# baumgach/PHiSeg-code

Hardware: AMD Instinct MI355X
Metric: training images/sec (ELBO step) phiseg_7_5 128x128 LIDC (higher is better)
Workload: dtype bf16; 1 GPU; phiseg_7_5 LIDC 128x128x1, 2 classes, bf16, batch norm, batch 64 per GPU, full ELBO training step (fwd + CE + KL + bwd + Adam); global_batch=64, parallelism=dp1

## Files before the change

### phiseg_code_amd/csrc/conv_c32.hip

```cpp
#include <stdlib.h>

#include <type_traits>

#include "phx_common.h"

namespace {

constexpr int C32_AI = 39;
constexpr int C32_NPL = 10;
constexpr int C32_STAGE = 40 * 1024;
constexpr int C32_PROW = 34 * 64;
constexpr int C32_LDS = 2 * C32_STAGE;

typedef __attribute__((address_space(3))) void* lds_ptr_t;

__device__ __forceinline__ unsigned lds_offset(const void* p) {
    return (unsigned)(uintptr_t)(const __attribute__((address_space(3))) unsigned char*)p;
}

__device__ unsigned long long* g_c32_trace = nullptr;
#define C32_TRACE(slot)                                                                          \
    do {                                                                                         \
        if (g_c32_trace && blockIdx.x == 0 && threadIdx.x == 0 && (slot) < 512)                   \
            g_c32_trace[slot] = __builtin_readcyclecounter();                                     \
    } while (0)

template <bool BIASACT, bool XF = false>
__global__ __launch_bounds__(256, 2) void k_conv3x3_c32(const unsigned short* __restrict__ x, const unsigned short* __restrict__ wpk,
                                                        unsigned short* __restrict__ y, const float* __restrict__ bias, int act,
                                                        float* __restrict__ stats_partial, int B, int H, int W, int tiles_x,
                                                        int tiles_y, int ntiles, const float* __restrict__ oscale, int stats_nrep, unsigned mgx, unsigned mgy,
                                                        const float* __restrict__ xscale = nullptr, const float* __restrict__ xshift = nullptr) {
    extern __shared__ __attribute__((aligned(16))) unsigned char smem[];
    const int wave = threadIdx.x >> 6, lane = threadIdx.x & 63;
    const int l31 = lane & 31, khalf = lane >> 5;

    bf16x8 fb[9][2];
#pragma unroll
    for (int tap = 0; tap < 9; ++tap)
#pragma unroll
        for (int ks = 0; ks < 2; ++ks)
            fb[tap][ks] = *reinterpret_cast<const bf16x8*>(wpk + ((tap * 32 + l31) * 32 + (ks * 2 + khalf) * 8));

    unsigned rel[C32_NPL], edge[C32_NPL];
#pragma unroll
    for (int n = 0; n < C32_NPL; ++n) {
        const int j = wave + 4 * n;
        const int e = j * 64 + lane, pp = e >> 2, slot = e & 3;
        const int py = pp / 34, px = pp - py * 34;
        rel[n] = (unsigned)((py * W + px) * 64 + ((slot ^ ((px >> 2) & 3)) << 4));
        edge[n] = (j < C32_AI && pp < 612) ? (unsigned)((px == 0) | ((px == 33) << 1) | ((py == 0) << 2) | ((py == 17) << 3)) : 15u;
    }
    const __amdgpu_buffer_rsrc_t rsx = __builtin_amdgcn_make_buffer_rsrc((void*)x, 0, (int)((unsigned)B * H * W * 64u), 0x00020000);
    auto decode = [&](int t, int* tx0, int* ty0, int* b0) {
        const int q1 = tiles_x == 1 ? t : (int)__umulhi((unsigned)t, mgx);
        *tx0 = (t - q1 * tiles_x) << 5;
// ... 248 lines not shown
```

### phiseg_code_amd/csrc/conv_wgrad.hip

```cpp
#include "conv_common.h"

template <int RB>
__device__ __forceinline__ int wswz(int pix, int byte_in_row) {
    if (RB == 128) return pix * 128 + (byte_in_row ^ (((pix >> 1) & 1) << 6));
    return pix * RB + byte_in_row;
}

template <int TCI, int TCO, bool BIGP, bool FAST16>
__device__ __forceinline__ void conv3x3_wgrad_body(const unsigned short* __restrict__ x0, const unsigned short* __restrict__ dy,
                                                   float* __restrict__ dw, float* __restrict__ ws, int B, int H, int W, int Cin,
                                                   int Cout, MTile g, int ntiles, int tiles_per_block, const int bx,
                                                   const int by, const int bz, const int gdx, const int gdy,
                                                   const unsigned short* __restrict__ x2 = nullptr, const int K1 = 0) {
    const bool src2 = x2 != nullptr && by * TCI >= K1;
    const unsigned short* __restrict__ x = src2 ? x2 : x0;
    const int xC = x2 == nullptr ? Cin : (src2 ? Cin - K1 : K1);
    const int xc0 = by * TCI - (src2 ? K1 : 0);
    constexpr int WI = TCI / 32, WJ = TCO / 32, WK = 4 / (WI * WJ);
    constexpr int RBX = TCI * 2, RBD = TCO * 2;
    constexpr int QX = TCI / 8, QD = TCO / 8;
    constexpr int NXI = ((BIGP ? 1024 : 400) * QX + 255) / 256;
    const int tw = 1 << g.tws, th = 1 << g.ths;
    const int pw = tw + 2, ph = th + 2;
    const int npatch = g.tb * ph * pw;
    extern __shared__ __attribute__((aligned(16))) unsigned char smem[];
    unsigned char* sX = smem;
    unsigned char* sD = smem + npatch * RBX;
    const int ci0 = by * TCI, co0 = bz * TCO;
    const int wave = threadIdx.x >> 6, lane = threadIdx.x & 63;
    const int wi = wave % WI, wj = (wave / WI) % WJ, wk = wave / (WI * WJ);
    const int c16 = lane & 15, cb16 = (lane >> 4) & 1, khalf = lane >> 5;
    const int chan_byte_x = (wi * 32 + cb16 * 16 + (c16 & 3) * 4) * 2;
    const int chan_byte_d = (wj * 32 + cb16 * 16 + (c16 & 3) * 4) * 2;
    typedef __attribute__((ext_vector_type(8))) short s16x8;
    unsigned dcon[2], xcon[2][3][2];
#pragma unroll
    for (int r = 0; r < 2; ++r) {
        const int lxr = khalf * 8 + r * 4 + (c16 >> 2);
        dcon[r] = (unsigned)wswz<RBD>(lxr, chan_byte_d);
#pragma unroll
// ... 65 lines not shown
        if constexpr (PHX_ABLATE & 16) return;
        if constexpr (idx < NXI) {
            const int gx = ptx0 + (planx[idx] & 255) - 1, gy = pty0 + ((planx[idx] >> 8) & 255) - 1, gb = pb0 + (planx[idx] >> 16);
            const bool ok = planx[idx] >= 0 && gx >= 0 && gx < W && gy >= 0 && gy < H && gb < B;
            const unsigned vo = ok ? (unsigned)(((gb * H + gy) * W + gx) * xC * 2 + qxb) : 0xffffffffu;
            rx[idx] = __builtin_amdgcn_raw_buffer_load_b128(rsx, vo, xc0 * 2, 0);
        } else if constexpr (idx < NXI + QD) {
            constexpr int it = idx - NXI;
            const int ox = ptx0 + (pland[it] & 255), oy = pty0 + ((pland[it] >> 8) & 255), ob = pb0 + (pland[it] >> 16);
            const bool ok = ox < W && oy < H && ob < B;
            const unsigned vo = ok ? (unsigned)(((ob * H + oy) * W + ox) * Cout * 2 + qdb) : 0xffffffffu;
            rd[it] = __builtin_amdgcn_raw_buffer_load_b128(rsd, vo, co0 * 2, 0);
        }
    };
    auto prefetch_range = [&](auto self, auto lo, auto hi) {
        constexpr int l = decltype(lo)::value, h = decltype(hi)::value;
        if constexpr (l < h && l < NXI + QD) {
            prefetch_piece(lo);
            self(self, std::integral_constant<int, l + 1>(), hi);
        }
    };
    const int t_begin = bx * tiles_per_block;
    const int t_end = min(ntiles, t_begin + tiles_per_block);
    PHX_BLOCKLOG_BEGIN();
    PHX_TRACE(0);
    if (t_begin < t_end) {
        if constexpr (FAST16) {
            decode(t_begin);
            prefetch_range(prefetch_range, std::integral_constant<int, 0>(), std::integral_constant<int, NXI + QD>());
        } else {
            prefetch(t_begin);
        }
    }
    PHX_TRACE(1);

    for (int t = t_begin; t < t_end; ++t) {
        __syncthreads();
        if (t == t_begin) PHX_TRACE(2);
#pragma unroll
        for (int it = 0; it < NXI; ++it) {
            const int i = threadIdx.x + it * 256;
            if (planx[it] >= 0) *reinterpret_cast<u32x4*>(sX + wswz<RBX>(i / QX, (i % QX) * 16)) = rx[it];
        }
#pragma unroll
        for (int it = 0; it < QD; ++it) {
            const int i = threadIdx.x + it * 256;
            *reinterpret_cast<u32x4*>(sD + wswz<RBD>(i / QD, (i % QD) * 16)) = rd[it];
        }
        __syncthreads();
        if (t == t_begin) PHX_TRACE(3);
        const bool more = t + 1 < t_end;
        if constexpr (FAST16) { if (more) decode(t + 1); }
        else if (more) prefetch(t + 1);
        if (t == t_begin) PHX_TRACE(4);
        if (FAST16) {
            constexpr int NSTEP = 16 / WK;
            s16x4 fd[2][2], fx[2][9][2];
            auto read_step = [&](unsigned xb, unsigned db, auto parc, auto bufc) {
                constexpr int P = decltype(parc)::value;
                constexpr int Bf = decltype(bufc)::value;
                fd[Bf][0] = __builtin_amdgcn_ds_read_tr16_b64_v4i16((s16x4 __attribute__((address_space(3)))*)(smem + db + dcon[0]));
                fd[Bf][1] = __builtin_amdgcn_ds_read_tr16_b64_v4i16((s16x4 __attribute__((address_space(3)))*)(smem + db + dcon[1]));
#pragma unroll
                for (int kh = 0; kh < 3; ++kh)
#pragma unroll
                    for (int kw = 0; kw < 3; ++kw) {
                        const int par = (P + kh) & 1;
                        fx[Bf][kh * 3 + kw][0] = __builtin_amdgcn_ds_read_tr16_b64_v4i16(
                            (s16x4 __attribute__((address_space(3)))*)(smem + xb + kh * 18 * RBX + xcon[0][kw][par]));
                        fx[Bf][kh * 3 + kw][1] = __builtin_amdgcn_ds_read_tr16_b64_v4i16(
                            (s16x4 __attribute__((address_space(3)))*)(smem + xb + kh * 18 * RBX + xcon[1][kw][par]));
                    }
            };
            auto mfma_step = [&](auto bufc) {
                constexpr int Bf = decltype(bufc)::value;
                const s16x8 dtmp = {fd[Bf][0][0], fd[Bf][0][1], fd[Bf][0][2], fd[Bf][0][3], fd[Bf][1][0], fd[Bf][1][1], fd[Bf][1][2], fd[Bf][1][3]};
                const bf16x8 bfrag = __builtin_bit_cast(bf16x8, dtmp);
// ... 46 lines not shown
                }
                const s16x4 d0 = __builtin_amdgcn_ds_read_tr16_b64_v4i16(
                    (s16x4 __attribute__((address_space(3)))*)(sD + wswz<RBD>(mpix[0], chan_byte_d)));
                const s16x4 d1 = __builtin_amdgcn_ds_read_tr16_b64_v4i16(
                    (s16x4 __attribute__((address_space(3)))*)(sD + wswz<RBD>(mpix[1], chan_byte_d)));
                const s16x8 dtmp = {d0[0], d0[1], d0[2], d0[3], d1[0], d1[1], d1[2], d1[3]};
                const bf16x8 bfrag = __builtin_bit_cast(bf16x8, dtmp);
    #pragma unroll
                for (int kh = 0; kh < 3; ++kh)
    #pragma unroll
                    for (int kw = 0; kw < 3; ++kw) {
                        const int sh = kh * pw + kw;
                        const s16x4 a0 = __builtin_amdgcn_ds_read_tr16_b64_v4i16(
                            (s16x4 __attribute__((address_space(3)))*)(sX + wswz<RBX>(ppix[0] + sh, chan_byte_x)));
                        const s16x4 a1 = __builtin_amdgcn_ds_read_tr16_b64_v4i16(
                            (s16x4 __attribute__((address_space(3)))*)(sX + wswz<RBX>(ppix[1] + sh, chan_byte_x)));
                        const s16x8 atmp = {a0[0], a0[1], a0[2], a0[3], a1[0], a1[1], a1[2], a1[3]};
                        const bf16x8 afrag = __builtin_bit_cast(bf16x8, atmp);
                        acc[kh * 3 + kw] = __builtin_amdgcn_mfma_f32_32x32x16_bf16(afrag, bfrag, acc[kh * 3 + kw], 0, 0, 0);
                    }
            }
        }
    }
    PHX_TRACE(5);
    if (ws) {
        const size_t cb = (size_t)bz * gdy + by;
        float* wp = ws + ((cb * gdx + bx) * WK + wk) * (size_t)(9 * TCI * TCO);
#pragma unroll
        for (int k = 0; k < 9; ++k)
#pragma unroll
            for (int r = 0; r < 16; ++r) {
                const int cil = wi * 32 + (r & 3) + 8 * (r >> 2) + 4 * (lane >> 5);
                wp[(k * TCI + cil) * TCO + wj * 32 + (lane & 31)] = acc[k][r];
            }
    } else {
        const int co = co0 + wj * 32 + (lane & 31);
#pragma unroll
        for (int k = 0; k < 9; ++k)
#pragma unroll
            for (int r = 0; r < 16; ++r) {
                const int ci = ci0 + wi * 32 + (r & 3) + 8 * (r >> 2) + 4 * (lane >> 5);
                atomicAdd(&dw[((size_t)k * Cin + ci) * Cout + co], acc[k][r]);
            }
    }
    PHX_TRACE(6);
    PHX_BLOCKLOG_END();
}

template <int TCI, int TCO, bool BIGP, bool FAST16>
__global__ __launch_bounds__(256, 1) void k_conv3x3_wgrad(const unsigned short* __restrict__ x,
                                                          const unsigned short* __restrict__ dy,
                                                          float* __restrict__ dw, float* __restrict__ ws, int B, int H,
                                                          int W, int Cin, int Cout, MTile g, int ntiles,
                                                          int tiles_per_block, const unsigned short* __restrict__ x2, int K1) {
    conv3x3_wgrad_body<TCI, TCO, BIGP, FAST16>(x, dy, dw, ws, B, H, W, Cin, Cout, g, ntiles, tiles_per_block, blockIdx.x,
                                               blockIdx.y, blockIdx.z, gridDim.x, gridDim.y, x2, K1);
}
struct WgMJob {
    const unsigned short* x; const unsigned short* dy; float* dw; float* ws;
    int B, H, W, Cin, Cout;
    MTile g;
    int ntiles, tpb, gdx, gdy, gdz, blk0;
    const unsigned short* x2; int K1, pad_;
};
template <int TCI, int TCO, bool BIGP>
__global__ __launch_bounds__(256, 1) void k_conv3x3_wgrad_multi(const WgMJob* __restrict__ jobs, int njobs) {
    int lo = 0, hi = njobs - 1;
    while (lo < hi) {
        const int mid = (lo + hi + 1) >> 1;
        if (jobs[mid].blk0 <= (int)blockIdx.x) lo = mid; else hi = mid - 1;
    }
    const WgMJob j = jobs[lo];
    const int local = blockIdx.x - j.blk0;
    conv3x3_wgrad_body<TCI, TCO, BIGP, false>(j.x, j.dy, j.dw, j.ws, j.B, j.H, j.W, j.Cin, j.Cout, j.g, j.ntiles, j.tpb,
                                              local % j.gdx, (local / j.gdx) % j.gdy, local / (j.gdx * j.gdy), j.gdx, j.gdy, j.x2, j.K1);
}

template <int TCI, int TCO>
__device__ __forceinline__ void conv3x3_wgrad_dma_body(const unsigned short* __restrict__ x0, const unsigned short* __restrict__ dy,
                                                       float* __restrict__ ws, int B, int H, int W, int Cin, int Cout, MTile g,
                                                       int ntiles, int tiles_per_block, const int bx, const int by, const int bz,
                                                       const int gdx, const int gdy,
                                                       const unsigned short* __restrict__ x2 = nullptr, const int K1 = 0,
                                                       const float* __restrict__ xscale = nullptr, const float* __restrict__ xshift = nullptr) {
    const bool src2 = x2 != nullptr && by * TCI >= K1;
    const unsigned short* __restrict__ x = src2 ? x2 : x0;
    const int xC = x2 == nullptr ? Cin : (src2 ? Cin - K1 : K1);
    const int xc0 = by * TCI - (src2 ? K1 : 0);
    constexpr int WI = TCI / 32, WJ = TCO / 32, WK = 4 / (WI * WJ);
    constexpr int RBX = TCI * 2, RBD = TCO * 2;
    constexpr int QX = TCI / 8, QD = TCO / 8;
    constexpr int NPATCH = 324;
    constexpr int XI = (NPATCH * QX + 63) / 64, DI = 256 * QD / 64;
    constexpr int XN = (XI + 3) / 4, DN = DI / 4;
    constexpr int SD_OFF = XI * 1024;
    extern __shared__ __attribute__((aligned(16))) unsigned char smem[];
    const int ci0 = by * TCI, co0 = bz * TCO;
    const int wave = threadIdx.x >> 6, lane = threadIdx.x & 63;
    const int wi = wave % WI, wj = (wave / WI) % WJ, wk = wave / (WI * WJ);
    const int c16 = lane & 15, cb16 = (lane >> 4) & 1, khalf = lane >> 5;
    const int chan_byte_x = (wi * 32 + cb16 * 16 + (c16 & 3) * 4) * 2;
    const int chan_byte_d = (wj * 32 + cb16 * 16 + (c16 & 3) * 4) * 2;
    typedef __attribute__((ext_vector_type(8))) short s16x8;
    unsigned dcon[2], xcon[2][3][2];
#pragma unroll
    for (int r = 0; r < 2; ++r) {
        const int lxr = khalf * 8 + r * 4 + (c16 >> 2);
        dcon[r] = (unsigned)(SD_OFF + wswz<RBD>(lxr, chan_byte_d));
#pragma unroll
        for (int kw = 0; kw < 3; ++kw)
#pragma unroll
            for (int par = 0; par < 2; ++par)
                xcon[r][kw][par] = (unsigned)((lxr + kw) * RBX +
                                              (RBX == 128 ? (chan_byte_x ^ (((((lxr + kw) >> 1) & 1) ^ par) << 6)) : chan_byte_x));
    }
    f32x16 acc[9];
#pragma unroll
    for (int k = 0; k < 9; ++k)
#pragma unroll
        for (int r = 0; r < 16; ++r) acc[k][r] = 0.f;

    constexpr bool RPLAN = WK == 1;
    auto plan_x = [&](int n) -> int {
        const int e = (wave + 4 * n) * 64 + lane;
        const int pp = e / QX, ps = e % QX;
        const int p = RBX == 128 ? (ps ^ (((pp >> 1) & 1) << 2)) : ps;
        return pp < NPATCH ? ((pp % 18) | ((pp / 18) << 8) | (p << 16)) : -1;
    };
    auto plan_d = [&](int n) -> int {
        const int e = (wave + 4 * n) * 64 + lane;
        const int m = e / QD, ps = e % QD;
        const int p = RBD == 128 ? (ps ^ (((m >> 1) & 1) << 2)) : ps;
        return (m & 15) | ((m >> 4) << 8) | (p << 16);
    };
    int planx[RPLAN ? XN : 1], pland[RPLAN ? DN : 1];
    if constexpr (RPLAN) {
#pragma unroll
        for (int n = 0; n < XN; ++n) planx[n] = plan_x(n);
#pragma unroll
        for (int n = 0; n < DN; ++n) pland[n] = plan_d(n);
    }
    const __amdgpu_buffer_rsrc_t rsx = __builtin_amdgcn_make_buffer_rsrc((void*)x, 0, (int)((unsigned)B * H * W * xC * 2u), 0x00020000);
    const __amdgpu_buffer_rsrc_t rsd = __builtin_amdgcn_make_buffer_rsrc((void*)dy, 0, (int)((unsigned)B * H * W * Cout * 2u), 0x00020000);
    typedef __attribute__((address_space(3))) void* lds_ptr_t;

    const int t_begin = bx * tiles_per_block;
    const int t_end = min(ntiles, t_begin + tiles_per_block);
    PHX_BLOCKLOG_BEGIN();
    for (int t = t_begin; t < t_end; ++t) {
        int tt = t;
        const int tx0 = (tt % g.tiles_x) << 4; tt /= g.tiles_x;
        const int ty0 = (tt % g.tiles_y) << 4; tt /= g.tiles_y;
        const int b0 = tt;
        __syncthreads();
#pragma unroll
        for (int n = 0; n < XN; ++n) {
            if (wave + 4 * n < XI) {
                int pk;
                if constexpr (RPLAN) pk = planx[n]; else pk = plan_x(n);
                const int gx = tx0 + (pk & 255) - 1, gy = ty0 + ((pk >> 8) & 255) - 1;
                const bool ok = pk >= 0 && gx >= 0 && gx < W && gy >= 0 && gy < H;
                const unsigned vo = ok ? (unsigned)((((b0 * H + gy) * W + gx) * xC) * 2 + (pk >> 16) * 16) : 0xffffffffu;
                __builtin_amdgcn_raw_ptr_buffer_load_lds(rsx, (lds_ptr_t)(smem + (wave + 4 * n) * 1024), 16, vo, xc0 * 2, 0, 0);
            }
        }
#pragma unroll
        for (int n = 0; n < DN; ++n) {
            int pk;
            if constexpr (RPLAN) pk = pland[n]; else pk = plan_d(n);
            const int ox = tx0 + (pk & 255), oy = ty0 + ((pk >> 8) & 255);
            const bool ok = ox < W && oy < H;
            const unsigned vo = ok ? (unsigned)((((b0 * H + oy) * W + ox) * Cout) * 2 + (pk >> 16) * 16) : 0xffffffffu;
            __builtin_amdgcn_raw_ptr_buffer_load_lds(rsd, (lds_ptr_t)(smem + SD_OFF + (wave + 4 * n) * 1024), 16, vo, co0 * 2, 0, 0);
        }
        asm volatile("s_waitcnt vmcnt(0)" ::: "memory");
        __syncthreads();
        if constexpr (TCI == 32) {
            if (xscale != nullptr) {
                typedef __attribute__((ext_vector_type(4))) unsigned u32x4_t;
                typedef __attribute__((ext_vector_type(4))) float f32x4_t;
                const int sp = threadIdx.x & 3;
                const f32x4_t c0 = *reinterpret_cast<const f32x4_t*>(xscale + ci0 + sp * 8), c1 = *reinterpret_cast<const f32x4_t*>(xscale + ci0 + sp * 8 + 4);
                const f32x4_t d0 = *reinterpret_cast<const f32x4_t*>(xshift + ci0 + sp * 8), d1 = *reinterpret_cast<const f32x4_t*>(xshift + ci0 + sp * 8 + 4);
                const float xsc[8] = {c0[0], c0[1], c0[2], c0[3], c1[0], c1[1], c1[2], c1[3]};
                const float xsh[8] = {d0[0], d0[1], d0[2], d0[3], d1[0], d1[1], d1[2], d1[3]};
#pragma unroll
                for (int n = 0; n < 6; ++n) {
                    const int pp = (int)(threadIdx.x >> 2) + 64 * n;
                    if (pp < NPATCH) {
                        const int py = (int)(((unsigned)pp * 3641u) >> 16), px = pp - py * 18;
                        const int gx = tx0 + px - 1, gy = ty0 + py - 1;
                        const bool inside = gx >= 0 && gx < W && gy >= 0 && gy < H;
                        u32x4_t* const q = reinterpret_cast<u32x4_t*>(smem + pp * RBX + sp * 16);
                        const u32x4_t r = *q;
                        u32x4_t o;
#pragma unroll
                        for (int k = 0; k < 4; ++k) {
                            const float a0 = fmaxf(fmaf(__uint_as_float(r[k] << 16), xsc[2 * k], xsh[2 * k]), 0.f);
                            const float a1 = fmaxf(fmaf(__uint_as_float(r[k] & 0xffff0000u), xsc[2 * k + 1], xsh[2 * k + 1]), 0.f);
                            o[k] = inside ? f2bf_pk(a0, a1) : 0u;
                        }
                        *q = o;
                    }
                }
                __syncthreads();
            }
        }

        constexpr int NSTEP = 16 / WK;
        s16x4 fd[2][2], fx[2][9][2];
        auto read_step = [&](unsigned xb, unsigned db, auto parc, auto bufc) {
            constexpr int P = decltype(parc)::value;
            constexpr int Bf = decltype(bufc)::value;
            fd[Bf][0] = __builtin_amdgcn_ds_read_tr16_b64_v4i16((s16x4 __attribute__((address_space(3)))*)(smem + db + dcon[0]));
            fd[Bf][1] = __builtin_amdgcn_ds_read_tr16_b64_v4i16((s16x4 __attribute__((address_space(3)))*)(smem + db + dcon[1]));
#pragma unroll
            for (int kh = 0; kh < 3; ++kh)
#pragma unroll
                for (int kw = 0; kw < 3; ++kw) {
                    const int par = (P + kh) & 1;
                    fx[Bf][kh * 3 + kw][0] = __builtin_amdgcn_ds_read_tr16_b64_v4i16(
                        (s16x4 __attribute__((address_space(3)))*)(smem + xb + kh * 18 * RBX + xcon[0][kw][par]));
                    fx[Bf][kh * 3 + kw][1] = __builtin_amdgcn_ds_read_tr16_b64_v4i16(
                        (s16x4 __attribute__((address_space(3)))*)(smem + xb + kh * 18 * RBX + xcon[1][kw][par]));
                }
        };
        auto mfma_step = [&](auto bufc) {
            constexpr int Bf = decltype(bufc)::value;
            const s16x8 dtmp = {fd[Bf][0][0], fd[Bf][0][1], fd[Bf][0][2], fd[Bf][0][3], fd[Bf][1][0], fd[Bf][1][1], fd[Bf][1][2], fd[Bf][1][3]};
            const bf16x8 bfrag = __builtin_bit_cast(bf16x8, dtmp);
#pragma unroll
            for (int k = 0; k < 9; ++k) {
                const s16x8 atmp = {fx[Bf][k][0][0], fx[Bf][k][0][1], fx[Bf][k][0][2], fx[Bf][k][0][3],
                                    fx[Bf][k][1][0], fx[Bf][k][1][1], fx[Bf][k][1][2], fx[Bf][k][1][3]};
                acc[k] = __builtin_amdgcn_mfma_f32_32x32x16_bf16(__builtin_bit_cast(bf16x8, atmp), bfrag, acc[k], 0, 0, 0);
            }
        };
        const unsigned xw = (unsigned)(wk * NSTEP * 18 * RBX), dw_ = (unsigned)(wk * NSTEP * 16 * RBD);
        read_step(xw, dw_, std::integral_constant<int, 0>(), std::integral_constant<int, 0>());
        auto steps = [&](auto self, auto stepc) {
            constexpr int SI = decltype(stepc)::value;
            if constexpr (SI < NSTEP) {
                if constexpr (SI + 1 < NSTEP)
                    read_step(xw + (SI + 1) * 18 * RBX, dw_ + (SI + 1) * 16 * RBD, std::integral_constant<int, (SI + 1) & 1>(),
                              std::integral_constant<int, (SI + 1) & 1>());
                mfma_step(std::integral_constant<int, SI & 1>());
                __builtin_amdgcn_sched_barrier(0);
                self(self, std::integral_constant<int, SI + 1>());
            }
        };
        steps(steps, std::integral_constant<int, 0>());
    }
    if constexpr (WK > 1) {
        typedef __attribute__((ext_vector_type(4))) float f32x4_t;
        f32x4_t* red = reinterpret_cast<f32x4_t*>(smem);
#pragma unroll
        for (int half = 1; half < WK; half <<= 1) {
            const int sel = wk & (2 * half - 1);
            f32x4_t* p = red + (size_t)(wi + WI * (wj + WJ * (wk / (2 * half)))) * (9 * 4 * 64) + lane;
            __syncthreads();
            if (sel == half)
#pragma unroll
                for (int k = 0; k < 9; ++k)
#pragma unroll
                    for (int q = 0; q < 4; ++q)
                        p[(k * 4 + q) * 64] = f32x4_t{acc[k][4 * q], acc[k][4 * q + 1], acc[k][4 * q + 2], acc[k][4 * q + 3]};
            __syncthreads();
            if (sel == 0)
#pragma unroll
                for (int k = 0; k < 9; ++k)
#pragma unroll
                    for (int q = 0; q < 4; ++q) {
                        const f32x4_t v = p[(k * 4 + q) * 64];
                        acc[k][4 * q] += v[0]; acc[k][4 * q + 1] += v[1]; acc[k][4 * q + 2] += v[2]; acc[k][4 * q + 3] += v[3];
                    }
        }
    }
    if (WK == 1 || wk == 0) {
        const size_t cb = (size_t)bz * gdy + by;
        float* wp = ws + (cb * gdx + bx) * (size_t)(9 * TCI * TCO);
#pragma unroll
        for (int k = 0; k < 9; ++k)
#pragma unroll
            for (int r = 0; r < 16; ++r) {
                const int cil = wi * 32 + (r & 3) + 8 * (r >> 2) + 4 * (lane >> 5);
                wp[(k * TCI + cil) * TCO + wj * 32 + (lane & 31)] = acc[k][r];
            }
    }
    PHX_BLOCKLOG_END();
}

template <int TCI, int TCO>
__global__ __launch_bounds__(256, 2) void k_conv3x3_wgrad_dma(const unsigned short* __restrict__ x,
                                                              const unsigned short* __restrict__ dy, float* __restrict__ ws,
                                                              int B, int H, int W, int Cin, int Cout, MTile g, int ntiles,
                                                              int tiles_per_block, const unsigned short* __restrict__ x2, int K1,
                                                              const float* __restrict__ xscale, const float* __restrict__ xshift) {
    conv3x3_wgrad_dma_body<TCI, TCO>(x, dy, ws, B, H, W, Cin, Cout, g, ntiles, tiles_per_block, blockIdx.x, blockIdx.y, blockIdx.z,
                                     gridDim.x, gridDim.y, x2, K1, xscale, xshift);
}
template <int TCI, int TCO>
__global__ __launch_bounds__(256, 2) void k_conv3x3_wgrad_dma_multi(const WgMJob* __restrict__ jobs, int njobs) {
    int lo = 0, hi = njobs - 1;
    while (lo < hi) {
        const int mid = (lo + hi + 1) >> 1;
        if (jobs[mid].blk0 <= (int)blockIdx.x) lo = mid; else hi = mid - 1;
    }
    const WgMJob j = jobs[lo];
    const int local = blockIdx.x - j.blk0;
    conv3x3_wgrad_dma_body<TCI, TCO>(j.x, j.dy, j.ws, j.B, j.H, j.W, j.Cin, j.Cout, j.g, j.ntiles, j.tpb, local % j.gdx,
                                     (local / j.gdx) % j.gdy, local / (j.gdx * j.gdy), j.gdx, j.gdy, j.x2, j.K1);
}

__device__ __forceinline__ void conv3x3_wgrad_pp_body(const unsigned short* __restrict__ x0, const unsigned short* __restrict__ dy,
                                                      float* __restrict__ ws, int B, int H, int W, int Cin, int Cout, MTile g,
                                                      int ntiles, int tiles_per_block, const int bx, const int by, const int bz,
                                                      const int gdx, const int gdy,
                                                      const unsigned short* __restrict__ x2 = nullptr, const int K1 = 0) {
    constexpr int TCI = 64, TCO = 64;
    const bool src2 = x2 != nullptr && by * TCI >= K1;
    const unsigned short* __restrict__ x = src2 ? x2 : x0;
    const int xC = x2 == nullptr ? Cin : (src2 ? Cin - K1 : K1);
    const int xc0 = by * TCI - (src2 ? K1 : 0);
    constexpr int RBX = 128, RBD = 128, QX = 8, QD = 8, NPATCH = 324;
    constexpr int XI = (NPATCH * QX + 63) / 64, DI = 256 * QD / 64;
    constexpr int XN = (XI + 3) / 4, DN = DI / 4;
    constexpr int SD_OFF = XI * 1024, STAGE = SD_OFF + 256 * RBD;
    extern __shared__ __attribute__((aligned(16))) unsigned char smem[];
    const int co0 = bz * TCO;
    const int wave = __builtin_amdgcn_readfirstlane((int)(threadIdx.x >> 6)), lane = threadIdx.x & 63;
    const int half = wave >> 2, lw = wave & 3;
    const int wi = lw & 1, wj = lw >> 1;
    const unsigned sbase = (unsigned)(half * STAGE);
    typedef __attribute__((ext_vector_type(8))) short s16x8;
    unsigned dcon[2], xcon[2][3][2];
    {
        const int c16 = lane & 15, cb16 = (lane >> 4) & 1, khalf = lane >> 5;
        const int chan_byte_x = (wi * 32 + cb16 * 16 + (c16 & 3) * 4) * 2;
        const int chan_byte_d = (wj * 32 + cb16 * 16 + (c16 & 3) * 4) * 2;
#pragma unroll
        for (int r = 0; r < 2; ++r) {
            const int lxr = khalf * 8 + r * 4 + (c16 >> 2);
// ... 79 lines not shown
                auto slot = [&](auto kc) {
                    constexpr int k = decltype(kc)::value, kh = k / 3, kw = k % 3, Rs = (SI + kh) & 3;
                    const s16x8 atmp = {fx[Rs][kw][0][0], fx[Rs][kw][0][1], fx[Rs][kw][0][2], fx[Rs][kw][0][3],
                                        fx[Rs][kw][1][0], fx[Rs][kw][1][1], fx[Rs][kw][1][2], fx[Rs][kw][1][3]};
                    acc[k] = __builtin_amdgcn_mfma_f32_32x32x16_bf16(__builtin_bit_cast(bf16x8, atmp), bfrag, acc[k], 0, 0, 0);
                    if constexpr (more) {
                        if constexpr (k < 2) rd_d(IC(SI + 1), kc);
                        else if constexpr (k < 8) rd_x(IC(SI + 3), IC((k - 2) >> 1), IC((k - 2) & 1));
                    }
                    __builtin_amdgcn_sched_barrier(0);
                };
                slot(IC(0)); slot(IC(1)); slot(IC(2)); slot(IC(3)); slot(IC(4)); slot(IC(5)); slot(IC(6)); slot(IC(7)); slot(IC(8));
                self(self, IC(SI + 1));
            }
        };
        steps(steps, IC(0));
#undef IC
    };
#define WPP_BARRIER() asm volatile("s_waitcnt vmcnt(0) lgkmcnt(0)\n\ts_barrier" ::: "memory")
    const int t_begin = bx * tiles_per_block;
    const int t_end = min(ntiles, t_begin + tiles_per_block);
    const int n = t_end - t_begin;
    const int nA = (n + 1) >> 1, nh = half ? (n >> 1) : nA;
    PHX_BLOCKLOG_BEGIN();
    if (half == 0 && nh > 0) load_tile(t_begin);
    WPP_BARRIER();
    if (half) {
        if (nh > 0) load_tile(t_begin + 1);
        WPP_BARRIER();
    }
    for (int k = 0; k < nA; ++k) {
        if (k < nh) compute();
        WPP_BARRIER();
        if (k + 1 < nh) load_tile(t_begin + half + 2 * (k + 1));
        WPP_BARRIER();
    }
    if (half == 0) WPP_BARRIER();
    typedef __attribute__((ext_vector_type(4))) float f32x4_t;
    f32x4_t* const pr = reinterpret_cast<f32x4_t*>(smem) + (size_t)lw * (9 * 4 * 64) + lane;
    if (half)
#pragma unroll
        for (int k = 0; k < 9; ++k)
#pragma unroll
            for (int q = 0; q < 4; ++q) pr[(k * 4 + q) * 64] = f32x4_t{acc[k][4 * q], acc[k][4 * q + 1], acc[k][4 * q + 2], acc[k][4 * q + 3]};
    WPP_BARRIER();
#undef WPP_BARRIER
    if (half == 0) {
        const size_t cb = (size_t)bz * gdy + by;
        float* wp = ws + (cb * gdx + bx) * (size_t)(9 * TCI * TCO);
#pragma unroll
        for (int k = 0; k < 9; ++k) {
#pragma unroll
            for (int q = 0; q < 4; ++q) {
                const f32x4_t v = pr[(k * 4 + q) * 64];
                acc[k][4 * q] += v[0]; acc[k][4 * q + 1] += v[1]; acc[k][4 * q + 2] += v[2]; acc[k][4 * q + 3] += v[3];
            }
#pragma unroll
            for (int r = 0; r < 16; ++r) {
                const int cil = wi * 32 + (r & 3) + 8 * (r >> 2) + 4 * (lane >> 5);
                wp[(k * TCI + cil) * TCO + wj * 32 + (lane & 31)] = acc[k][r];
            }
        }
    }
    PHX_BLOCKLOG_END();
}

__global__ __launch_bounds__(512, 1) void k_conv3x3_wgrad_pp(const unsigned short* __restrict__ x, const unsigned short* __restrict__ dy,
                                                             float* __restrict__ ws, int B, int H, int W, int Cin, int Cout, MTile g,
                                                             int ntiles, int tiles_per_block, const unsigned short* __restrict__ x2,
                                                             int K1) {
    conv3x3_wgrad_pp_body(x, dy, ws, B, H, W, Cin, Cout, g, ntiles, tiles_per_block, blockIdx.x, blockIdx.y, blockIdx.z, gridDim.x,
                          gridDim.y, x2, K1);
}
__global__ __launch_bounds__(512, 1) void k_conv3x3_wgrad_pp_multi(const WgMJob* __restrict__ jobs, int njobs) {
    int lo = 0, hi = njobs - 1;
    while (lo < hi) {
        const int mid = (lo + hi + 1) >> 1;
        if (jobs[mid].blk0 <= (int)blockIdx.x) lo = mid; else hi = mid - 1;
    }
    const WgMJob j = jobs[lo];
    const int local = blockIdx.x - j.blk0;
    const int cb = j.gdy * j.gdz, t = local >> 3;
    const int c = t % cb, bx = (t / cb) * 8 + (local & 7);
    if (bx >= j.gdx) return;
    conv3x3_wgrad_pp_body(j.x, j.dy, j.ws, j.B, j.H, j.W, j.Cin, j.Cout, j.g, j.ntiles, j.tpb, bx, c % j.gdy, c / j.gdy, j.gdx, j.gdy,
                          j.x2, j.K1);
}
// ... 42 lines not shown
    int lo = 0, hi = njobs - 1;
    while (lo < hi) {
        const int mid = (lo + hi + 1) >> 1;
        if (jobs[mid].blk0 <= (int)blockIdx.x) lo = mid; else hi = mid - 1;
    }
    const WgrJob j = jobs[lo];
    const int local = blockIdx.x - j.blk0;
    wgrad_reduce_body(j.ws, j.dw, j.nslice, j.Cin, j.Cout, j.tci, j.tco, local % j.gx, local / j.gx, j.gy);
}


int phx_wgrad_set_debug(void* trace_buf, void* blocklog_buf, int which) {
    unsigned long long* p = (unsigned long long*)(which == 0 ? trace_buf : blocklog_buf);
    if (which == 0) PHX_CHECK_HIP(hipMemcpyToSymbol(HIP_SYMBOL(g_phx_trace), &p, sizeof(p)));
    else PHX_CHECK_HIP(hipMemcpyToSymbol(HIP_SYMBOL(g_phx_blocklog), &p, sizeof(p)));
    return PHX_OK;
}

extern "C" {

static bool wgrad_dma_enabled() { return true; }
static size_t wgrad_dma_lds(int tci, int tco) {
    if (tci == 64 && tco == 64) return (size_t)2 * (41 * 1024 + 256 * 128);
    const size_t stage = (size_t)((324 * (tci / 8) + 63) / 64) * 1024 + (size_t)256 * tco * 2;
    const size_t red = (tci == 64 && tco == 64) ? 0 : (size_t)2 * 9 * 16 * 64 * sizeof(float);
    return stage > red ? stage : red;
}
static int wgrad_plan(int B, int H, int W, int Cin, int Cout, MTile* g, int* tci, int* tco, int* gx, int* tpb, int* wk,
                      int target_override = 0, int K1 = 0) {
    *g = make_mtile(B, H, W);
    const int ntiles = g->tiles_x * g->tiles_y * g->tiles_b;
    *tci = Cin % 64 == 0 ? 64 : 32;
    if (K1 > 0 && K1 % 64 != 0) *tci = 32;
    *tco = Cout % 64 == 0 ? 64 : 32;
    *wk = 4 / ((*tci / 32) * (*tco / 32));
    if (wgrad_dma_enabled() && g->tws == 4 && g->ths == 4 && g->tb == 1) *wk = 1;
    const int cblocks = (Cin / *tci) * (Cout / *tco);
    int target_blocks = cblocks <= 4 && *tci == 64 && *tco == 64 ? 512 : 384;
    if (ntiles <= 256 && target_blocks > 256) target_blocks = 256;
    const bool pp = wgrad_dma_enabled() && g->tws == 4 && g->ths == 4 && g->tb == 1 && *tci == 64 && *tco == 64;
    if (pp) target_blocks = 256;
    if (target_override > 0) target_blocks = pp ? (target_override + 1) / 2 : target_override;
    int split = (target_blocks + cblocks - 1) / cblocks;
    if (pp && target_override <= 0) split = target_blocks / cblocks;
    if (pp && target_override > 0) {
        const int alone = 256 / cblocks > 0 ? 256 / cblocks : 1;
        split = (split + 7) & ~7;
// ... 239 lines not shown
```

Baseline: 6756 images/s.

## Double-buffer DMA wgrad tiles and tighten LDS addressing with immediate offsets

New measurement: 6807 images/s, median of 6. Within noise of the previous version (+0.8%).

```diff
diff --git a/phiseg_code_amd/csrc/conv_c32.hip b/phiseg_code_amd/csrc/conv_c32.hip
--- a/phiseg_code_amd/csrc/conv_c32.hip
+++ b/phiseg_code_amd/csrc/conv_c32.hip
@@ -21,8 +21,7 @@
 __device__ unsigned long long* g_c32_trace = nullptr;
 #define C32_TRACE(slot)                                                                          \
     do {                                                                                         \
-        if (g_c32_trace && blockIdx.x == 0 && threadIdx.x == 0 && (slot) < 512)                   \
-            g_c32_trace[slot] = __builtin_readcyclecounter();                                     \
+        if (trc != nullptr && threadIdx.x == 0 && (slot) < 512) trc[slot] = __builtin_readcyclecounter(); \
     } while (0)
 
 template <bool BIASACT, bool XF = false>
@@ -32,6 +31,7 @@
                                                         int tiles_y, int ntiles, const float* __restrict__ oscale, int stats_nrep, unsigned mgx, unsigned mgy,
                                                         const float* __restrict__ xscale = nullptr, const float* __restrict__ xshift = nullptr) {
     extern __shared__ __attribute__((aligned(16))) unsigned char smem[];
+    unsigned long long* const trc = blockIdx.x == 0 ? g_c32_trace : nullptr;
     const int wave = threadIdx.x >> 6, lane = threadIdx.x & 63;
     const int l31 = lane & 31, khalf = lane >> 5;
 
diff --git a/phiseg_code_amd/csrc/conv_wgrad.hip b/phiseg_code_amd/csrc/conv_wgrad.hip
--- a/phiseg_code_amd/csrc/conv_wgrad.hip
+++ b/phiseg_code_amd/csrc/conv_wgrad.hip
@@ -16,6 +16,9 @@
     const unsigned short* __restrict__ x = src2 ? x2 : x0;
     const int xC = x2 == nullptr ? Cin : (src2 ? Cin - K1 : K1);
     const int xc0 = by * TCI - (src2 ? K1 : 0);
+    const unsigned long long trv = (unsigned long long)g_phx_trace, blv = (unsigned long long)g_phx_blocklog;
+    asm volatile("" ::: "memory");
+    unsigned long long *trc = nullptr, *blg = nullptr;
     constexpr int WI = TCI / 32, WJ = TCO / 32, WK = 4 / (WI * WJ);
     constexpr int RBX = TCI * 2, RBD = TCO * 2;
     constexpr int QX = TCI / 8, QD = TCO / 8;
@@ -127,8 +130,7 @@
     };
     const int t_begin = bx * tiles_per_block;
     const int t_end = min(ntiles, t_begin + tiles_per_block);
-    PHX_BLOCKLOG_BEGIN();
-    PHX_TRACE(0);
+    const unsigned long long bl_t0 = __builtin_readcyclecounter();
     if (t_begin < t_end) {
         if constexpr (FAST16) {
             decode(t_begin);
@@ -137,11 +139,14 @@
             prefetch(t_begin);
         }
     }
-    PHX_TRACE(1);
+    blg = phx_uniform_ptr(blv);
+    trc = (blockIdx.x | blockIdx.y | blockIdx.z) == 0 ? phx_uniform_ptr(trv) : nullptr;
+    PHX_TRACE_TO(trc, 0, bl_t0);
+    PHX_TRACE_TO(trc, 1, __builtin_readcyclecounter());
 
     for (int t = t_begin; t < t_end; ++t) {
         __syncthreads();
-        if (t == t_begin) PHX_TRACE(2);
+        if (t == t_begin) PHX_TRACE_TO(trc, 2, __builtin_readcyclecounter());
 #pragma unroll
         for (int it = 0; it < NXI; ++it) {
             const int i = threadIdx.x + it * 256;
@@ -153,11 +158,11 @@
             *reinterpret_cast<u32x4*>(sD + wswz<RBD>(i / QD, (i % QD) * 16)) = rd[it];
         }
         __syncthreads();
-        if (t == t_begin) PHX_TRACE(3);
+        if (t == t_begin) PHX_TRACE_TO(trc, 3, __builtin_readcyclecounter());
         const bool more = t + 1 < t_end;
         if constexpr (FAST16) { if (more) decode(t + 1); }
         else if (more) prefetch(t + 1);
-        if (t == t_begin) PHX_TRACE(4);
+        if (t == t_begin) PHX_TRACE_TO(trc, 4, __builtin_readcyclecounter());
         if (FAST16) {
             constexpr int NSTEP = 16 / WK;
             s16x4 fd[2][2], fx[2][9][2];
@@ -250,7 +255,7 @@
             }
         }
     }
-    PHX_TRACE(5);
+    PHX_TRACE_TO(trc, 5, __builtin_readcyclecounter());
     if (ws) {
         const size_t cb = (size_t)bz * gdy + by;
         float* wp = ws + ((cb * gdx + bx) * WK + wk) * (size_t)(9 * TCI * TCO);
@@ -271,8 +276,8 @@
                 atomicAdd(&dw[((size_t)k * Cin + ci) * Cout + co], acc[k][r]);
             }
     }
-    PHX_TRACE(6);
-    PHX_BLOCKLOG_END();
+    PHX_TRACE_TO(trc, 6, __builtin_readcyclecounter());
+    PHX_BLOCKLOG_END_TO(blg);
 }
 
 template <int TCI, int TCO, bool BIGP, bool FAST16>
@@ -304,6 +309,18 @@
                                               local % j.gdx, (local / j.gdx) % j.gdy, local / (j.gdx * j.gdy), j.gdx, j.gdy, j.x2, j.K1);
 }
 
+#ifndef PHX_WGRAD_DMA_STAGES
+#define PHX_WGRAD_DMA_STAGES 0
+#endif
+constexpr int wgrad_dma_xstages(int tci, int tco) {
+    return PHX_WGRAD_DMA_STAGES == 1 ? 1 : PHX_WGRAD_DMA_STAGES == 2 ? 2 : PHX_WGRAD_DMA_STAGES == 3 ? (tci == 32 ? 2 : 1) : (tci == 32 && tco == 32 ? 2 : 1);
+}
+constexpr int wgrad_dma_dstages(int tci, int tco) {
+    return PHX_WGRAD_DMA_STAGES == 1 ? 1 : PHX_WGRAD_DMA_STAGES == 2 ? 2 : PHX_WGRAD_DMA_STAGES == 3 ? (tco == 32 ? 2 : 1) : (tci == 32 && tco == 32 ? 2 : 1);
+}
+__device__ __forceinline__ unsigned wg_lds_offset(const void* p) {
+    return (unsigned)(uintptr_t)(const __attribute__((address_space(3))) unsigned char*)p;
+}
 template <int TCI, int TCO>
 __device__ __forceinline__ void conv3x3_wgrad_dma_body(const unsigned short* __restrict__ x0, const unsigned short* __restrict__ dy,
                                                        float* __restrict__ ws, int B, int H, int W, int Cin, int Cout, MTile g,
@@ -321,26 +338,33 @@
     constexpr int NPATCH = 324;
     constexpr int XI = (NPATCH * QX + 63) / 64, DI = 256 * QD / 64;
     constexpr int XN = (XI + 3) / 4, DN = DI / 4;
-    constexpr int SD_OFF = XI * 1024;
+    constexpr int XS = wgrad_dma_xstages(TCI, TCO), DS = wgrad_dma_dstages(TCI, TCO);
+    constexpr bool PIPE = XS == 2 || DS == 2;
+    constexpr int XSTAGE = XI * 1024, DSTAGE = 256 * RBD;
+    constexpr int SD_OFF = XS * XSTAGE;
     extern __shared__ __attribute__((aligned(16))) unsigned char smem[];
+    const unsigned long long blv = (unsigned long long)g_phx_blocklog;
+    asm volatile("" ::: "memory");
     const int ci0 = by * TCI, co0 = bz * TCO;
-    const int wave = threadIdx.x >> 6, lane = threadIdx.x & 63;
+    const int wave = __builtin_amdgcn_readfirstlane((int)(threadIdx.x >> 6)), lane = threadIdx.x & 63;
     const int wi = wave % WI, wj = (wave / WI) % WJ, wk = wave / (WI * WJ);
     const int c16 = lane & 15, cb16 = (lane >> 4) & 1, khalf = lane >> 5;
     const int chan_byte_x = (wi * 32 + cb16 * 16 + (c16 & 3) * 4) * 2;
     const int chan_byte_d = (wj * 32 + cb16 * 16 + (c16 & 3) * 4) * 2;
     typedef __attribute__((ext_vector_type(8))) short s16x8;
+    constexpr int NSTEP = 16 / WK;
+    const unsigned lds0 = wg_lds_offset(smem);
     unsigned dcon[2], xcon[2][3][2];
 #pragma unroll
     for (int r = 0; r < 2; ++r) {
         const int lxr = khalf * 8 + r * 4 + (c16 >> 2);
-        dcon[r] = (unsigned)(SD_OFF + wswz<RBD>(lxr, chan_byte_d));
+        dcon[r] = lds0 + (unsigned)(SD_OFF + wk * NSTEP * 16 * RBD + wswz<RBD>(lxr, chan_byte_d));
 #pragma unroll
         for (int kw = 0; kw < 3; ++kw)
 #pragma unroll
             for (int par = 0; par < 2; ++par)
-                xcon[r][kw][par] = (unsigned)((lxr + kw) * RBX +
-                                              (RBX == 128 ? (chan_byte_x ^ (((((lxr + kw) >> 1) & 1) ^ par) << 6)) : chan_byte_x));
+                xcon[r][kw][par] = lds0 + (unsigned)(wk * NSTEP * 18 * RBX + (lxr + kw) * RBX +
+                                                     (RBX == 128 ? (chan_byte_x ^ (((((lxr + kw) >> 1) & 1) ^ par) << 6)) : chan_byte_x));
     }
     f32x16 acc[9];
 #pragma unroll
@@ -348,79 +372,116 @@
 #pragma unroll
         for (int r = 0; r < 16; ++r) acc[k][r] = 0.f;
 
-    constexpr bool RPLAN = WK == 1;
-    auto plan_x = [&](int n) -> int {
-        const int e = (wave + 4 * n) * 64 + lane;
-        const int pp = e / QX, ps = e % QX;
-        const int p = RBX == 128 ? (ps ^ (((pp >> 1) & 1) << 2)) : ps;
-        return pp < NPATCH ? ((pp % 18) | ((pp / 18) << 8) | (p << 16)) : -1;
-    };
-    auto plan_d = [&](int n) -> int {
-        const int e = (wave + 4 * n) * 64 + lane;
-        const int m = e / QD, ps = e % QD;
-        const int p = RBD == 128 ? (ps ^ (((m >> 1) & 1) << 2)) : ps;
-        return (m & 15) | ((m >> 4) << 8) | (p << 16);
-    };
-    int planx[RPLAN ? XN : 1], pland[RPLAN ? DN : 1];
-    if constexpr (RPLAN) {
-#pragma unroll
-        for (int n = 0; n < XN; ++n) planx[n] = plan_x(n);
-#pragma unroll
-        for (int n = 0; n < DN; ++n) pland[n] = plan_d(n);
-    }
     const __amdgpu_buffer_rsrc_t rsx = __builtin_amdgcn_make_buffer_rsrc((void*)x, 0, (int)((unsigned)B * H * W * xC * 2u), 0x00020000);
     const __amdgpu_buffer_rsrc_t rsd = __builtin_amdgcn_make_buffer_rsrc((void*)dy, 0, (int)((unsigned)B * H * W * Cout * 2u), 0x00020000);
     typedef __attribute__((address_space(3))) void* lds_ptr_t;
 
-    const int t_begin = bx * tiles_per_block;
-    const int t_end = min(ntiles, t_begin + tiles_per_block);
-    PHX_BLOCKLOG_BEGIN();
-    for (int t = t_begin; t < t_end; ++t) {
+    auto issue_x = [&](int t, int xs) __attribute__((always_inline)) {
+        unsigned ln = lane;
+        asm volatile("" : "+v"(ln));
         int tt = t;
         const int tx0 = (tt % g.tiles_x) << 4; tt /= g.tiles_x;
         const int ty0 = (tt % g.tiles_y) << 4; tt /= g.tiles_y;
-        const int b0 = tt;
-        __syncthreads();
+        const unsigned sbase = (unsigned)tt * (unsigned)(H * W * xC * 2) + (unsigned)(xc0 * 2);
+        const unsigned lp = ln / QX, ps = ln % QX;
 #pragma unroll
         for (int n = 0; n < XN; ++n) {
             if (wave + 4 * n < XI) {
-                int pk;
-                if constexpr (RPLAN) pk = planx[n]; else pk = plan_x(n);
-                const int gx = tx0 + (pk & 255) - 1, gy = ty0 + ((pk >> 8) & 255) - 1;
-                const bool ok = pk >= 0 && gx >= 0 && gx < W && gy >= 0 && gy < H;
-                const unsigned vo = ok ? (unsigned)((((b0 * H + gy) * W + gx) * xC) * 2 + (pk >> 16) * 16) : 0xffffffffu;
-                __builtin_amdgcn_raw_ptr_buffer_load_lds(rsx, (lds_ptr_t)(smem + (wave + 4 * n) * 1024), 16, vo, xc0 * 2, 0, 0);
-            }
-        }
+                const unsigned pp = (unsigned)((wave + 4 * n) * (64 / QX)) + lp;
+                const unsigned p = RBX == 128 ? (ps ^ (((pp >> 1) & 1u) << 2)) : ps;
+                const unsigned py = __umul24(pp, 3641u) >> 16, px = pp - __umul24(py, 18u);
+                const unsigned gx = (unsigned)(tx0 - 1) + px, gy = (unsigned)(ty0 - 1) + py;
+                const bool ok = pp < (unsigned)NPATCH && gx < (unsigned)W && gy < (unsigned)H;
+                const unsigned off = __umul24(__umul24(gy, (unsigned)W) + gx, (unsigned)(xC * 2)) + p * 16u;
+                const unsigned vo = off | (ok ? 0u : 0xffffffffu);
+                __builtin_amdgcn_raw_ptr_buffer_load_lds(rsx, (lds_ptr_t)(smem + xs * XSTAGE + (wave + 4 * n) * 1024), 16, vo, sbase, 0, 0);
+            }
+        }
+    };
+    auto issue_d = [&](int t, int ds) __attribute__((always_inline)) {
+        unsigned ln = lane;
+        asm volatile("" : "+v"(ln));
+        int tt = t;
+        const int tx0 = (tt % g.tiles_x) << 4; tt /= g.tiles_x;
+        const int ty0 = (tt % g.tiles_y) << 4; tt /= g.tiles_y;
+        const unsigned sbase = (unsigned)tt * (unsigned)(H * W * Cout * 2) + (unsigned)(co0 * 2);
+        const unsigned lm = ln / QD, ps = ln % QD;
 #pragma unroll
         for (int n = 0; n < DN; ++n) {
-            int pk;
-            if constexpr (RPLAN) pk = pland[n]; else pk = plan_d(n);
-            const int ox = tx0 + (pk & 255), oy = ty0 + ((pk >> 8) & 255);
-            const bool ok = ox < W && oy < H;
-            const unsigned vo = ok ? (unsigned)((((b0 * H + oy) * W + ox) * Cout) * 2 + (pk >> 16) * 16) : 0xffffffffu;
-            __builtin_amdgcn_raw_ptr_buffer_load_lds(rsd, (lds_ptr_t)(smem + SD_OFF + (wave + 4 * n) * 1024), 16, vo, co0 * 2, 0, 0);
-        }
-        asm volatile("s_waitcnt vmcnt(0)" ::: "memory");
-        __syncthreads();
+            const unsigned m = (unsigned)((wave + 4 * n) * (64 / QD)) + lm;
+            const unsigned p = RBD == 128 ? (ps ^ (((m >> 1) & 1u) << 2)) : ps;
+            const unsigned ox = (unsigned)tx0 + (m & 15u), oy = (unsigned)ty0 + (m >> 4);
+            const bool ok = ox < (unsigned)W && oy < (unsigned)H;
+            const unsigned off = __umul24(__umul24(oy, (unsigned)W) + ox, (unsigned)(Cout * 2)) + p * 16u;
+            const unsigned vo = off | (ok ? 0u : 0xffffffffu);
+            __builtin_amdgcn_raw_ptr_buffer_load_lds(rsd, (lds_ptr_t)(smem + SD_OFF + ds * DSTAGE + (wave + 4 * n) * 1024), 16, vo, sbase, 0, 0);
+        }
+    };
+    typedef __attribute__((ext_vector_type(4))) unsigned u32x4_t;
+    typedef __attribute__((ext_vector_type(4))) float f32x4_t;
+    constexpr int COEF_OFF = SD_OFF + DS * DSTAGE;
+
+    const int t_begin = bx * tiles_per_block;
+    const int t_end = min(ntiles, t_begin + tiles_per_block);
+    const unsigned long long bl_t0 = __builtin_readcyclecounter();
+    if (t_begin < t_end) {
+        if constexpr (XS == 2) issue_x(t_begin, 0);
+        if constexpr (DS == 2) issue_d(t_begin, 0);
+    }
+    unsigned long long* const blg = phx_uniform_ptr(blv);
+    if constexpr (TCI == 32) {
+        if (xscale != nullptr && threadIdx.x < 64)
+            reinterpret_cast<float*>(smem + COEF_OFF)[threadIdx.x] = threadIdx.x < 32 ? xscale[ci0 + threadIdx.x] : xshift[ci0 + threadIdx.x - 32];
+    }
+    for (int t = t_begin, it = 0; t < t_end; ++t, ++it) {
+        const int cur = it & 1;
+        const bool more = t + 1 < t_end;
+        asm volatile("s_waitcnt vmcnt(0) lgkmcnt(0)\n\ts_barrier" ::: "memory");
+        if constexpr (XS == 1) issue_x(t, 0);
+        if constexpr (DS == 1) issue_d(t, 0);
+        if (more) {
+            if constexpr (XS == 2) issue_x(t + 1, cur ^ 1);
+            if constexpr (DS == 2) issue_d(t + 1, cur ^ 1);
+        }
+        if constexpr (XS == 1 || DS == 1) {
+            if constexpr (!PIPE) {
+                asm volatile("s_waitcnt vmcnt(0)" ::: "memory");
+            } else if (!more) {
+                asm volatile("s_waitcnt vmcnt(0)" ::: "memory");
+            } else if constexpr (XS == 2) {
+                if (wave < XI - 4 * (XN - 1)) asm volatile("s_waitcnt vmcnt(%0)" ::"n"(XN) : "memory");
+                else asm volatile("s_waitcnt vmcnt(%0)" ::"n"(XN - 1) : "memory");
+            } else {
+                asm volatile("s_waitcnt vmcnt(%0)" ::"n"(DN) : "memory");
+            }
+            asm volatile("s_barrier" ::: "memory");
+        }
         if constexpr (TCI == 32) {
             if (xscale != nullptr) {
-                typedef __attribute__((ext_vector_type(4))) unsigned u32x4_t;
-                typedef __attribute__((ext_vector_type(4))) float f32x4_t;
-                const int sp = threadIdx.x & 3;
-                const f32x4_t c0 = *reinterpret_cast<const f32x4_t*>(xscale + ci0 + sp * 8), c1 = *reinterpret_cast<const f32x4_t*>(xscale + ci0 + sp * 8 + 4);
-                const f32x4_t d0 = *reinterpret_cast<const f32x4_t*>(xshift + ci0 + sp * 8), d1 = *reinterpret_cast<const f32x4_t*>(xshift + ci0 + sp * 8 + 4);
+                const unsigned xst = XS == 2 ? (unsigned)(cur * XSTAGE) : 0u;
+                int tt = t;
+                const int tx0 = (tt % g.tiles_x) << 4; tt /= g.tiles_x;
+                const int ty0 = (tt % g.tiles_y) << 4;
+                int tid = threadIdx.x;
+                asm volatile("" : "+v"(tid));
+                const int sp = tid & 3;
+                f32x4_t c0, c1, d0, d1;
+                asm volatile("ds_read_b128 %0, %4\n\tds_read_b128 %1, %4 offset:16\n\tds_read_b128 %2, %4 offset:128\n\t"
+                             "ds_read_b128 %3, %4 offset:144\n\ts_waitcnt lgkmcnt(0)"
+                             : "=&v"(c0), "=&v"(c1), "=&v"(d0), "=&v"(d1) : "v"(lds0 + (unsigned)(COEF_OFF + sp * 32)) : "memory");
                 const float xsc[8] = {c0[0], c0[1], c0[2], c0[3], c1[0], c1[1], c1[2], c1[3]};
                 const float xsh[8] = {d0[0], d0[1], d0[2], d0[3], d1[0], d1[1], d1[2], d1[3]};
 #pragma unroll
-                for (int n = 0; n < 6; ++n) {
-                    const int pp = (int)(threadIdx.x >> 2) + 64 * n;
-                    if (pp < NPATCH) {
+                for (int n = 0; n < 6; n += 2) {
+                    const int ppa = (tid >> 2) + 64 * n, ppb = ppa + 64;
+                    const bool vb = ppb < NPATCH;
+                    const unsigned qa = lds0 + xst + (unsigned)(ppa * RBX + sp * 16), qb = lds0 + xst + (unsigned)((vb ? ppb : ppa) * RBX + sp * 16);
+                    u32x4_t ra, rb;
+                    asm volatile("ds_read_b128 %0, %2\n\tds_read_b128 %1, %3\n\ts_waitcnt lgkmcnt(0)" : "=&v"(ra), "=&v"(rb) : "v"(qa), "v"(qb) : "memory");
+                    auto form = [&](int pp, const u32x4_t r) -> u32x4_t {
                         const int py = (int)(((unsigned)pp * 3641u) >> 16), px = pp - py * 18;
                         const int gx = tx0 + px - 1, gy = ty0 + py - 1;
                         const bool inside = gx >= 0 && gx < W && gy >= 0 && gy < H;
-                        u32x4_t* const q = reinterpret_cast<u32x4_t*>(smem + pp * RBX + sp * 16);
-                        const u32x4_t r = *q;
                         u32x4_t o;
 #pragma unroll
                         for (int k = 0; k < 4; ++k) {
@@ -428,56 +489,91 @@
                             const float a1 = fmaxf(fmaf(__uint_as_float(r[k] & 0xffff0000u), xsc[2 * k + 1], xsh[2 * k + 1]), 0.f);
                             o[k] = inside ? f2bf_pk(a0, a1) : 0u;
                         }
-                        *q = o;
-                    }
+                        return o;
+                    };
+                    const u32x4_t oa = form(ppa, ra), ob = form(ppb, rb);
+                    asm volatile("ds_write_b128 %0, %1" ::"v"(qa), "v"(oa) : "memory");
+                    if (vb) asm volatile("ds_write_b128 %0, %1" ::"v"(qb), "v"(ob) : "memory");
                 }
-                __syncthreads();
-            }
-        }
-
-        constexpr int NSTEP = 16 / WK;
+                asm volatile("s_waitcnt lgkmcnt(0)\n\ts_barrier" ::: "memory");
+            }
+        }
+
         s16x4 fd[2][2], fx[2][9][2];
-        auto read_step = [&](unsigned xb, unsigned db, auto parc, auto bufc) {
-            constexpr int P = decltype(parc)::value;
-            constexpr int Bf = decltype(bufc)::value;
-            fd[Bf][0] = __builtin_amdgcn_ds_read_tr16_b64_v4i16((s16x4 __attribute__((address_space(3)))*)(smem + db + dcon[0]));
-            fd[Bf][1] = __builtin_amdgcn_ds_read_tr16_b64_v4i16((s16x4 __attribute__((address_space(3)))*)(smem + db + dcon[1]));
+        auto trd = [&](unsigned a, auto immc) __attribute__((always_inline)) -> s16x4 {
+            constexpr int imm = decltype(immc)::value;
+            static_assert(imm >= 0 && imm < 65536, "ds offset field");
+            if constexpr (PIPE) {
+                s16x4 v;
+                asm volatile("ds_read_b64_tr_b16 %0, %1 offset:%2" : "=v"(v) : "v"(a), "n"(imm));
+                return v;
+            } else {
+                return __builtin_amdgcn_ds_read_tr16_b64_v4i16((s16x4 __attribute__((address_space(3)))*)(uintptr_t)(a + imm));
+            }
+        };
+        auto read_step = [&](auto stepc) __attribute__((always_inline)) {
+            constexpr int SI = decltype(stepc)::value, P = SI & 1, Bf = SI & 1;
+            fd[Bf][0] = trd(dcon[0], std::integral_constant<int, SI * 16 * RBD>());
+            fd[Bf][1] = trd(dcon[1], std::integral_constant<int, SI * 16 * RBD>());
 #pragma unroll
             for (int kh = 0; kh < 3; ++kh)
 #pragma unroll
                 for (int kw = 0; kw < 3; ++kw) {
                     const int par = (P + kh) & 1;
-                    fx[Bf][kh * 3 + kw][0] = __builtin_amdgcn_ds_read_tr16_b64_v4i16(
-                        (s16x4 __attribute__((address_space(3)))*)(smem + xb + kh * 18 * RBX + xcon[0][kw][par]));
-                    fx[Bf][kh * 3 + kw][1] = __builtin_amdgcn_ds_read_tr16_b64_v4i16(
-                        (s16x4 __attribute__((address_space(3)))*)(smem + xb + kh * 18 * RBX + xcon[1][kw][par]));
+                    const unsigned a0 = xcon[0][kw][par], a1 = xcon[1][kw][par];
+                    auto rd2 = [&](auto khc) __attribute__((always_inline)) {
+                        constexpr int imm = (SI + decltype(khc)::value) * 18 * RBX;
+                        fx[Bf][kh * 3 + kw][0] = trd(a0, std::integral_constant<int, imm>());
+                        fx[Bf][kh * 3 + kw][1] = trd(a1, std::integral_constant<int, imm>());
+                    };
+                    if (kh == 0) rd2(std::integral_constant<int, 0>());
+                    else if (kh == 1) rd2(std::integral_constant<int, 1>());
+                    else rd2(std::integral_constant<int, 2>());
                 }
         };
-        auto mfma_step = [&](auto bufc) {
+        auto mfma_one = [&](auto bufc, int k) __attribute__((always_inline)) {
             constexpr int Bf = decltype(bufc)::value;
             const s16x8 dtmp = {fd[Bf][0][0], fd[Bf][0][1], fd[Bf][0][2], fd[Bf][0][3], fd[Bf][1][0], fd[Bf][1][1], fd[Bf][1][2], fd[Bf][1][3]};
-            const bf16x8 bfrag = __builtin_bit_cast(bf16x8, dtmp);
-#pragma unroll
-            for (int k = 0; k < 9; ++k) {
-                const s16x8 atmp = {fx[Bf][k][0][0], fx[Bf][k][0][1], fx[Bf][k][0][2], fx[Bf][k][0][3],
-                                    fx[Bf][k][1][0], fx[Bf][k][1][1], fx[Bf][k][1][2], fx[Bf][k][1][3]};
-                acc[k] = __builtin_amdgcn_mfma_f32_32x32x16_bf16(__builtin_bit_cast(bf16x8, atmp), bfrag, acc[k], 0, 0, 0);
-            }
+            const s16x8 atmp = {fx[Bf][k][0][0], fx[Bf][k][0][1], fx[Bf][k][0][2], fx[Bf][k][0][3],
+                                fx[Bf][k][1][0], fx[Bf][k][1][1], fx[Bf][k][1][2], fx[Bf][k][1][3]};
+            acc[k] = __builtin_amdgcn_mfma_f32_32x32x16_bf16(__builtin_bit_cast(bf16x8, atmp), __builtin_bit_cast(bf16x8, dtmp), acc[k], 0, 0, 0);
         };
-        const unsigned xw = (unsigned)(wk * NSTEP * 18 * RBX), dw_ = (unsigned)(wk * NSTEP * 16 * RBD);
-        read_step(xw, dw_, std::integral_constant<int, 0>(), std::integral_constant<int, 0>());
+        read_step(std::integral_constant<int, 0>());
         auto steps = [&](auto self, auto stepc) {
             constexpr int SI = decltype(stepc)::value;
             if constexpr (SI < NSTEP) {
-                if constexpr (SI + 1 < NSTEP)
-                    read_step(xw + (SI + 1) * 18 * RBX, dw_ + (SI + 1) * 16 * RBD, std::integral_constant<int, (SI + 1) & 1>(),
-                              std::integral_constant<int, (SI + 1) & 1>());
-                mfma_step(std::integral_constant<int, SI & 1>());
+                if constexpr (PIPE) {
+                    asm volatile("s_waitcnt lgkmcnt(0)" ::: "memory");
+                    __builtin_amdgcn_sched_barrier(0);
+                    mfma_one(std::integral_constant<int, SI & 1>(), 0);
+                    __builtin_amdgcn_sched_barrier(0);
+                    if constexpr (SI + 1 < NSTEP) read_step(std::integral_constant<int, SI + 1>());
+                    __builtin_amdgcn_sched_barrier(0);
+#pragma unroll
+                    for (int k = 1; k < 9; ++k) mfma_one(std::integral_constant<int, SI & 1>(), k);
+                } else {
+                    if constexpr (SI + 1 < NSTEP) read_step(std::integral_constant<int, SI + 1>());
+#pragma unroll
+                    for (int k = 0; k < 9; ++k) mfma_one(std::integral_constant<int, SI & 1>(), k);
+                }
                 __builtin_amdgcn_sched_barrier(0);
                 self(self, std::integral_constant<int, SI + 1>());
             }
         };
         steps(steps, std::integral_constant<int, 0>());
+        if constexpr (XS == 2) {
+            const unsigned dx = cur ? (unsigned)-XSTAGE : (unsigned)XSTAGE;
+#pragma unroll
+            for (int r = 0; r < 2; ++r)
+#pragma unroll
+                for (int kw = 0; kw < 3; ++kw)
+#pragma unroll
+                    for (int par = 0; par < 2; ++par) xcon[r][kw][par] += dx;
+        }
+        if constexpr (DS == 2) {
+            const unsigned dd = cur ? (unsigned)-DSTAGE : (unsigned)DSTAGE;
+            dcon[0] += dd; dcon[1] += dd;
+        }
     }
     if constexpr (WK > 1) {
         typedef __attribute__((ext_vector_type(4))) float f32x4_t;
@@ -515,7 +611,7 @@
                 wp[(k * TCI + cil) * TCO + wj * 32 + (lane & 31)] = acc[k][r];
             }
     }
-    PHX_BLOCKLOG_END();
+    PHX_BLOCKLOG_END_TO(blg);
 }
 
 template <int TCI, int TCO>
@@ -546,6 +642,8 @@
                                                       const int gdx, const int gdy,
                                                       const unsigned short* __restrict__ x2 = nullptr, const int K1 = 0) {
     constexpr int TCI = 64, TCO = 64;
+    const unsigned long long blv = (unsigned long long)g_phx_blocklog;
+    asm volatile("" ::: "memory");
     const bool src2 = x2 != nullptr && by * TCI >= K1;
     const unsigned short* __restrict__ x = src2 ? x2 : x0;
     const int xC = x2 == nullptr ? Cin : (src2 ? Cin - K1 : K1);
@@ -671,8 +769,9 @@
     const int t_end = min(ntiles, t_begin + tiles_per_block);
     const int n = t_end - t_begin;
     const int nA = (n + 1) >> 1, nh = half ? (n >> 1) : nA;
-    PHX_BLOCKLOG_BEGIN();
+    const unsigned long long bl_t0 = __builtin_readcyclecounter();
     if (half == 0 && nh > 0) load_tile(t_begin);
+    unsigned long long* const blg = phx_uniform_ptr(blv);
     WPP_BARRIER();
     if (half) {
         if (nh > 0) load_tile(t_begin + 1);
@@ -711,7 +810,7 @@
             }
         }
     }
-    PHX_BLOCKLOG_END();
+    PHX_BLOCKLOG_END_TO(blg);
 }
 
 __global__ __launch_bounds__(512, 1) void k_conv3x3_wgrad_pp(const unsigned short* __restrict__ x, const unsigned short* __restrict__ dy,
@@ -800,7 +899,8 @@
 static bool wgrad_dma_enabled() { return true; }
 static size_t wgrad_dma_lds(int tci, int tco) {
     if (tci == 64 && tco == 64) return (size_t)2 * (41 * 1024 + 256 * 128);
-    const size_t stage = (size_t)((324 * (tci / 8) + 63) / 64) * 1024 + (size_t)256 * tco * 2;
+    const size_t stage = (size_t)wgrad_dma_xstages(tci, tco) * ((324 * (tci / 8) + 63) / 64) * 1024 + (size_t)wgrad_dma_dstages(tci, tco) * 256 * tco * 2 +
+                         (tci == 32 ? 256 : 0);
     const size_t red = (tci == 64 && tco == 64) ? 0 : (size_t)2 * 9 * 16 * 64 * sizeof(float);
     return stage > red ? stage : red;
 }
```
